# bbc/vc2-reference

Hardware: AMD Instinct MI355X
Metric: Mpixels/s encode+decode, UHD-1 10-bit HQ_ConstQ (higher is better)
Workload: dtype int32; 1 GPU; BASELINE cfg2: UHD-1 3840x2160 4:2:2 10-bit HQ_ConstQ DD97 depth 4, -u 1 -a 2 -q 16 -S 2; streams=1, parallelism=frame-parallel x1, no collective

## Files before the change

vc2-reference_amd/csrc/vc2hip_slices.hip:

```cpp
#include <stdlib.h>

#include <algorithm>
#include <atomic>
#include <mutex>

#include "vc2hip_internal.h"
#include "vc2hip_store.h"

void vc2_prof_begin(Launcher &L, const char *name, hipStream_t s);
void vc2_prof_end(Launcher &L, hipStream_t s);

__constant__ QuantTables c_qs;
void vc2_upload_p16_tables(const QuantTables &t, hipStream_t s);
void vc2_upload_tables_slices(const QuantTables &t, hipStream_t s) {
  (void)hipMemcpyToSymbolAsync(HIP_SYMBOL(c_qs), &t, sizeof t, 0, hipMemcpyHostToDevice, s);
  vc2_upload_p16_tables(t, s);
}

__device__ __forceinline__ int quant_core(int v, int qf, unsigned mg, int sh) {
  const unsigned mag = v < 0 ? 0u - (unsigned)v : (unsigned)v;
  const int a = (int)(mag << 2);
  const unsigned t = __umulhi(mg, (unsigned)a);
  int q = (int)((t + (((unsigned)a - t) >> 1)) >> sh);
  const bool slow = !(qf > 1 && a >= 0);
// ... 1946 lines not shown
      for (int c = 0; c < comp; ++c) at += 1 + (unsigned long long)rd(at) * p.scalar;
      len = rd(at) * p.scalar;
      at += 1;
      if (at + len > plen) {
        atomicOr(p.err, VC2_DEVERR_STREAM);
        len = at < plen ? (unsigned)(plen - at) : 0;
      }
      pos = at < plen ? (unsigned)at : 0u;
    }
#ifdef VC2HIP_ABLATE
    br.dbg_mask = VC2_SKIP(p, 1) ? 0x3FFCu : ~0u;
#endif
    br.safe = (unsigned)min((unsigned long long)p.payload_stride + mis, 0xFFFFFFF0ull);
    br.init(pay, pos + mis, (int)len);
  }
#pragma unroll
  for (int k = 0; k < UNP_PITCH; k += 8) *(int4 *)(st + k) = make_int4(0, 0, 0, 0);
  __syncthreads();
  int cnt = 0;
  signed char *sb = (signed char *)st;
  auto byte_of = [&](int j, int v) __attribute__((always_inline)) -> int {
    if (__builtin_expect((unsigned)(v + 127) <= 254u, 1)) return v;
    escape(j, v);
    if (p.stats) {
      const uint2 pc = *(const uint2 *)(sb + (cnt & ~7));
      auto has80 = [](unsigned x) -> bool { const unsigned y = x ^ 0x80808080u; return ((y - 0x01010101u) & ~y & 0x80808080u) != 0u; };
      if (!has80(pc.x) && !has80(pc.y)) atomicAdd(p.stats, 1ull);
    }
    return -128;
  };
  auto turns = [&](auto bytes, const int base, const int room) __attribute__((always_inline)) {
    constexpr bool BY = decltype(bytes)::value;
    for (int turn = 0; cnt < room; ++turn) {
      int used = 0;
#pragma unroll
      for (int look = 0; look < UNP_LOOKS; ++look) {
        const unsigned w = look ? (unsigned)((br.acc << used) >> 32) : br.top();
        unsigned e = lut[w >> (32 - UNP_LUT_BITS)];
#if VC2_UNP_BRANCHLESS
        if (look) e = (cnt < room && (look < 3 || used + UNP_LUT_BITS <= br.have)) ? e : 0u;
#else
        if (e != 0 && (look == 0 || (used != 0 && cnt < room)))
#endif
        {
          if constexpr (BY) {
            sb[cnt + (int)((e >> 8) & 15u)] = (signed char)(e >> 16);
            sb[cnt + (int)((e >> 12) & 15u)] = (signed char)(e >> 24);
          } else {
            st[cnt + (int)((e >> 8) & 15u)] = (short)__builtin_amdgcn_sbfe((int)e, 16, 8);
            st[cnt + (int)((e >> 12) & 15u)] = (short)((int)e >> 24);
          }
          cnt += (int)((e >> 4) & 15u);
          used += (int)(e & 15u);
        }
      }
      if ((turn & UNP_LONG_EVERY) == UNP_LONG_EVERY) {
        if (used == 0 && cnt < room) {
          const unsigned hi = br.top();
          const unsigned follow = hi & 0xAAAAAAAAu;
          if (follow != 0) {
            const int K = __clz((int)follow) >> 1;
            const unsigned body = hi >> ((32 - 2 * K) & 31);
            const unsigned mag = ((1u << K) | compact_even32(body)) - 1u;
            const int neg = (int)((hi >> ((30 - 2 * K) & 31)) & 1u);
            int v = neg ? (int)(0u - mag) : (int)mag;
            if constexpr (BY) { v = byte_of(base + cnt, v); sb[cnt++] = (signed char)v; }
            else {
              if (!St<int16_t>::fits(v)) { escape(base + cnt, v); v = VC2_ST_SENTINEL; }
              st[cnt++] = (short)v;
            }
            used = 2 * K + 2;
          } else {
            unsigned value = 1;
            for (;;) {
              const unsigned f = br.top() >> 31;
              br.skip(pay, 1);
              if (f) break;
              value = (value << 1) | (br.top() >> 31);
              br.skip(pay, 1);
            }
            value -= 1u;
            int v = 0;
            if (value) {
              v = (br.top() >> 31) ? (int)(0u - value) : (int)value;
              br.skip(pay, 1);
            }
            if constexpr (BY) { v = byte_of(base + cnt, v); sb[cnt++] = (signed char)v; }
            else {
              if (!St<int16_t>::fits(v)) { escape(base + cnt, v); v = VC2_ST_SENTINEL; }
              st[cnt++] = (short)v;
            }
          }
        }
      }
      br.skip(pay, used);
    }
  };
  const int n16 = BP8 ? min(n, p.bp.from[comp]) : n;
  int base = 0;
  for (; base < n16; base += UNP_N) {
    const int room = min(UNP_N, n - base);
    turns(std::false_type(), base, room);
    wave_lds_sync();
    const short *sw = stage[wave];
    typedef int v4i __attribute__((ext_vector_type(4)));
    typedef int v2i __attribute__((ext_vector_type(2)));
    const int rec_end = VC2_SKIP(p, 2) ? room : min(room, p.bp.from[comp] - base);
    if (rec_end > 0 && !VC2_SKIP(p, 2)) {
#pragma unroll
      for (int j = 0; j < PR; ++j) {
        const int r = j * (64 / PR) + lane / PR, c = (lane % PR) * 8;
        if (slice0 + r < p.n_slices && c < rec_end) {
          const int4 v = *(const int4 *)(sw + r * UNP_PITCH + c);
          const v4i vv = {v.x, v.y, v.z, v.w};
          int16_t *dst = (int16_t *)p.store + rec0 + (size_t)(slice0 + r) * p.slice_coefs + base + c;
          if (base + c < p.hs.n[comp])
            dst = (int16_t *)p.store + (size_t)pic * p.store_stride + (size_t)p.hs.base[comp] + (size_t)(slice0 + r) * p.hs.n[comp] + base + c;
          __builtin_nontemporal_store(vv, (__attribute__((address_space(1))) v4i *)(size_t)dst);
        }
      }
    }
    if (rec_end < room) {
      for (int q = 0; q < PR;) {
        const int j0 = base + 8 * q;
        if (8 * q >= room) break;
        if (j0 < p.bp.from[comp]) { ++q; continue; }
        int lw, ow, lbase;
        int at = band_plane_at(p.bp, comp, n, j0, sy, sx, lw, ow, &lbase);
        if (!active) at = -1;
        lw = __builtin_amdgcn_readfirstlane(lw);
        const int lp = lw - 3, P = lw >= 4 ? 1 << lp : 1;
        if (lw >= 4 && q + P <= PR && ((j0 >> 3) & (P - 1)) == 0) {
          for (int k = 0; k < P; ++k) {
            const int t = lane + 64 * k, sl = t >> lp, pp = t & (P - 1);
            const int at_t = __shfl(at, sl);
            if (at_t >= 0) {
              const int4 v = *(const int4 *)(sw + sl * UNP_PITCH + 8 * (q + pp));
              if constexpr (BP8) {
                const uint2 b8 = unp_bytes8(v, p.store_wide + (size_t)pic * p.store_stride, at_t + 8 * pp, 0, p.stats);
                const v2i vb = {(int)b8.x, (int)b8.y};
                char *dst = (char *)((int16_t *)p.store + (size_t)pic * p.store_stride) + (size_t)(at_t + 8 * pp) + (size_t)lbase;
                __builtin_nontemporal_store(vb, (__attribute__((address_space(1))) v2i *)(size_t)dst);
              } else {
              const v4i vv = {v.x, v.y, v.z, v.w};
              int16_t *dst = (int16_t *)p.store + (size_t)pic * p.store_stride + (size_t)(at_t + 8 * pp);
              __builtin_nontemporal_store(vv, (__attribute__((address_space(1))) v4i *)(size_t)dst);
              }
            }
          }
          q += P;
          continue;
        }
        if (BP8 && at >= 0) {
          const int4 v = *(const int4 *)(st + 8 * q);
          char *dst = (char *)((int16_t *)p.store + (size_t)pic * p.store_stride) + (size_t)at + (size_t)lbase;
          const uint2 b8 = unp_bytes8(v, p.store_wide + (size_t)pic * p.store_stride, at, lw >= 3 ? 0 : ow, p.stats);
          if (lw >= 3) {
            const v2i vb = {(int)b8.x, (int)b8.y};
            __builtin_nontemporal_store(vb, (__attribute__((address_space(1))) v2i *)(size_t)dst);
          } else {
            __builtin_nontemporal_store((int)b8.x, (__attribute__((address_space(1))) int *)(size_t)dst);
            __builtin_nontemporal_store((int)b8.y, (__attribute__((address_space(1))) int *)(size_t)(dst + ow));
          }
        } else if (at >= 0) {
          int16_t *dst = (int16_t *)p.store + (size_t)pic * p.store_stride + (size_t)at;
          const int4 v = *(const int4 *)(st + 8 * q);
          if (lw >= 3) {
            const v4i vv = {v.x, v.y, v.z, v.w};
            __builtin_nontemporal_store(vv, (__attribute__((address_space(1))) v4i *)(size_t)dst);
          } else {
            const v2i lo = {v.x, v.y}, hi = {v.z, v.w};
            __builtin_nontemporal_store(lo, (__attribute__((address_space(1))) v2i *)(size_t)dst);
            __builtin_nontemporal_store(hi, (__attribute__((address_space(1))) v2i *)(size_t)(dst + ow));
          }
        }
        ++q;
      }
    }
    wave_lds_sync();
    const int4 spill = *(const int4 *)(st + UNP_N);
#pragma unroll
    for (int k = 0; k < UNP_PITCH; k += 8) *(int4 *)(st + k) = make_int4(0, 0, 0, 0);
    cnt = max(cnt - UNP_N, 0);
    if (cnt) *(int4 *)st = spill;
  }
  if constexpr (BP8) {
    constexpr int UNB_N = 2 * UNP_N, UNB_PR = UNB_N / 8, UNB_PITCH = 2 * UNP_PITCH;
    static_assert(UNB_N + 8 <= UNB_PITCH, "a byte row and its slack fit the lane's part of the stage");
    if (base < n) {
      const int4 c16 = *(const int4 *)st;
      *(int4 *)st = make_int4((int)__builtin_amdgcn_perm((unsigned)c16.y, (unsigned)c16.x, 0x06040200u),
                              (int)__builtin_amdgcn_perm((unsigned)c16.w, (unsigned)c16.z, 0x06040200u), 0, 0);
    }
    const char *sw8 = (const char *)stage[wave];
    char *planes = (char *)((int16_t *)p.store + (size_t)pic * p.store_stride);
    typedef int v2i __attribute__((ext_vector_type(2)));
    for (; base < n; base += UNB_N) {
      const int room = min(UNB_N, n - base);
      turns(std::true_type(), base, room);
      wave_lds_sync();
      for (int q = 0; q < UNB_PR;) {
        if (8 * q >= room) break;
        const int j0 = base + 8 * q;
        int lw, ow, lbase;
        int at = band_plane_at(p.bp, comp, n, j0, sy, sx, lw, ow, &lbase);
        if (!active) at = -1;
        lw = __builtin_amdgcn_readfirstlane(lw);
        const int lp = lw - 3, P = lw >= 4 ? 1 << lp : 1;
        if (lw >= 4 && q + P <= UNB_PR && ((j0 >> 3) & (P - 1)) == 0) {
          for (int k = 0; k < P; ++k) {
            const int t = lane + 64 * k, sl = t >> lp, pp = t & (P - 1);
            const int at_t = __shfl(at, sl);
            if (at_t >= 0) {
              const v2i vb = *(const v2i *)(sw8 + sl * UNB_PITCH + 8 * (q + pp));
              __builtin_nontemporal_store(vb, (__attribute__((address_space(1))) v2i *)(size_t)(planes + (size_t)(at_t + 8 * pp) + (size_t)lbase));
            }
          }
          q += P;
          continue;
        }
        if (at >= 0) {
          const v2i vb = *(const v2i *)(sb + 8 * q);
          char *dst = planes + (size_t)at + (size_t)lbase;
          if (lw >= 3) __builtin_nontemporal_store(vb, (__attribute__((address_space(1))) v2i *)(size_t)dst);
          else {
            __builtin_nontemporal_store(vb.x, (__attribute__((address_space(1))) int *)(size_t)dst);
            __builtin_nontemporal_store(vb.y, (__attribute__((address_space(1))) int *)(size_t)(dst + ow));
          }
        }
        ++q;
      }
      wave_lds_sync();
      const v2i spill = *(const v2i *)(sb + UNB_N);
#pragma unroll
      for (int k = 0; k < UNB_PITCH; k += 16) *(int4 *)(sb + k) = make_int4(0, 0, 0, 0);
      cnt = max(cnt - UNB_N, 0);
      if (cnt) *(v2i *)sb = spill;
    }
  }
}

void vc2_launch_unpack(Launcher &L, const UnpackParams &p0, int n_pictures, hipStream_t s) {
  UnpackParams p = p0;
#ifdef VC2HIP_ABLATE
  { const char *e = getenv("VC2HIP_DEBUG_UNPACK"); p.debug_skip = e ? atoi(e) : 0; }
#endif
  if (!p.bp.levels) for (int c = 0; c < 3; ++c) p.bp.from[c] = 1 << 30;
  if (p.xs < 1) p.xs = 1;
  vc2_prof_begin(L, "hq_unpack", s);
  if (p.store16) {
    constexpr int T = 64 * VC2_UNP16_WAVES;
    const int nblk = (p.n_slices + T - 1) / T;
    const bool b8 = p.bp.levels && p.bp.bytes8;
#if VC2_UNP_ORDER == 2
    if (b8) VC2_LAUNCH(L, k_hq_unpack16<true>, dim3(nblk, n_pictures, 3), dim3(T), 0, s, p);
    else VC2_LAUNCH(L, k_hq_unpack16<false>, dim3(nblk, n_pictures, 3), dim3(T), 0, s, p);
#else
    if (b8) VC2_LAUNCH(L, k_hq_unpack16<true>, dim3(((nblk + 7) / 8) * 8 * 3, n_pictures), dim3(T), 0, s, p);
    else VC2_LAUNCH(L, k_hq_unpack16<false>, dim3(((nblk + 7) / 8) * 8 * 3, n_pictures), dim3(T), 0, s, p);
#endif
    vc2_prof_end(L, s);
    return;
  }
  static const int wide = vc2_tune_int("VC2HIP_UNPACK_WIDE", 1);
  static const int nt = vc2_tune_int("VC2HIP_UNPACK_NT", 1);
  if (!nt) VC2_LAUNCH(L, (k_hq_unpack<16, false>), dim3((p.n_slices + 255) / 256, n_pictures, 3), dim3(256), 0, s, p);
  else if (wide) VC2_LAUNCH(L, k_hq_unpack<32>, dim3((p.n_slices + 255) / 256, n_pictures, 3), dim3(256), 0, s, p);
  else VC2_LAUNCH(L, k_hq_unpack<16>, dim3((p.n_slices + 255) / 256, n_pictures, 3), dim3(256), 0, s, p);
  vc2_prof_end(L, s);
}

static int idx_chunk(int E) { return E <= 1024 ? 8192 : E <= 8191 ? 16384 : 32768; }

__device__ __forceinline__ int slice_len_lds(const uint8_t *b, int pos, int prefix, int scalar) {
  int q = pos + prefix + 1;
  q += 1 + b[q] * scalar;
  q += 1 + b[q] * scalar;
  q += 1 + b[q] * scalar;
  return q - pos;
}

__device__ void stage_chunk(uint8_t *lds, const uint8_t *pay, unsigned long long plen,
                            unsigned long long c0, int nbytes) {
  for (int i = threadIdx.x * 16; i < nbytes; i += blockDim.x * 16) {
    uint4 v = make_uint4(0, 0, 0, 0);
    const unsigned long long a = c0 + i;
    if (a + 16 <= plen) v = *(const uint4 *)(pay + a);
    else {
      unsigned w[4] = {0, 0, 0, 0};
      for (int k = 0; k < 16; ++k) if (a + k < plen) w[k >> 2] |= (unsigned)pay[a + k] << (8 * (k & 3));
      v = make_uint4(w[0], w[1], w[2], w[3]);
    }
    *(uint4 *)(lds + i) = v;
  }
}

static constexpr int IDX_MAX_E = 32767;
constexpr int idx_threads(int CH, int GS = 0) { return (CH >> GS) <= 8192 ? 512 : 1024; }

template <int CH, int GS>
__global__ __launch_bounds__(idx_threads(CH, GS)) void k_index_tables_nx(const uint8_t *payload, long long stride,
                                                                 const unsigned long long *lens, unsigned *tables,
                                                                 int n_chunks, int E, int prefix, int scalar, unsigned *err, const unsigned *skip,
                                                                 int merge) {
  constexpr int NT = idx_threads(CH, GS), NP = CH >> GS;
  if (skip && *skip == 0) return;
  extern __shared__ __attribute__((aligned(16))) uint8_t lds_b[];
  const int chunk = blockIdx.x, pic = blockIdx.y;
  if (chunk == 0 && threadIdx.x == 0 && lens[pic] > (unsigned long long)stride) atomicOr(err, VC2_DEVERR_STREAM);
  const unsigned long long plen = min(lens[pic], (unsigned long long)stride), c0 = (unsigned long long)chunk * CH;
  if (c0 >= plen) return;
  const int nbytes = (CH + E + 16 + 15) & ~15;
  const int EU = E >> GS;
  unsigned short *nx = (unsigned short *)(lds_b + nbytes);
  stage_chunk(lds_b, payload + (size_t)pic * stride, plen, c0, nbytes);
  __syncthreads();
  const int lim = (int)min((unsigned long long)CH, plen - c0);
  constexpr int PER = NP / NT;
  {
    int q[PER];
#pragma unroll
    for (int k = 0; k < PER; ++k) q[k] = ((threadIdx.x + k * NT) << GS) + prefix + 1;
#pragma unroll
    for (int c = 0; c < 3; ++c) {
      int len[PER];
#pragma unroll
      for (int k = 0; k < PER; ++k) len[k] = lds_b[min(q[k], nbytes - 1)];
#pragma unroll
      for (int k = 0; k < PER; ++k) q[k] += 1 + len[k] * scalar;
    }
#pragma unroll
    for (int k = 0; k < PER; ++k) {
      const int n = q[k];
      nx[threadIdx.x + k * NT] = (unsigned short)(n >= lim ? (n >= CH ? n : CH) : n);
    }
  }
  __syncthreads();
  unsigned *tab = tables + ((size_t)pic * n_chunks + chunk) * EU;
  if (!merge) {
    for (int e = threadIdx.x; e < EU; e += NT) {
      int pos = e << GS, cnt = 0;
      if (pos >= lim) pos = CH;
      while (pos < CH) { pos = nx[pos >> GS]; ++cnt; }
      tab[e] = (unsigned)(pos - CH) << 16 | (unsigned)cnt;
    }
    return;
  }
  unsigned *W = (unsigned *)(nx + NP);
  unsigned *need = W + EU;
  unsigned short *list = (unsigned short *)(need + (EU + 31) / 32);
  __shared__ unsigned s_count;
  for (int t = threadIdx.x; t < (EU + 31) / 32; t += NT) need[t] = 0;
  if (threadIdx.x == 0) s_count = 0;
  __syncthreads();
  constexpr int EPT = 4096 / NT;
  int la[EPT], ca[EPT];
#pragma unroll
  for (int k = 0; k < EPT; ++k) {
    const int e = threadIdx.x + k * NT;
    la[k] = CH; ca[k] = 0;
    if (e < EU && (e << GS) < lim) {
      int pos = e << GS, cnt = 0;
      while (pos < E) { pos = nx[pos >> GS]; ++cnt; }
      la[k] = pos; ca[k] = cnt;
      if (pos < CH) {
        const int t = (pos - E) >> GS;
        if (!(atomicOr(&need[t >> 5], 1u << (t & 31)) >> (t & 31) & 1u)) list[atomicAdd(&s_count, 1u)] = (unsigned short)t;
      }
    }
  }
  __syncthreads();
  for (int i = threadIdx.x; i < (int)s_count; i += NT) {
    const int t = list[i];
    int pos = E + (t << GS), cnt = 0;
    while (pos < CH) { pos = nx[pos >> GS]; ++cnt; }
    W[t] = (unsigned)(pos - CH) << 16 | (unsigned)cnt;
  }
  __syncthreads();
#pragma unroll
  for (int k = 0; k < EPT; ++k) {
    const int e = threadIdx.x + k * NT;
    if (e >= EU) continue;
    if (la[k] >= CH) tab[e] = (unsigned)(la[k] - CH) << 16 | (unsigned)ca[k];
    else tab[e] = W[(la[k] - E) >> GS] + (unsigned)ca[k];
  }
}

static constexpr int IDX_GROUP = 16;

template <bool WORD> __device__ __forceinline__ uint2 idx_entry(const void *tab, size_t i) {
  if constexpr (WORD) { const unsigned t = ((const unsigned *)tab)[i]; return make_uint2(t >> 16, t & 0xFFFFu); }
  else return ((const uint2 *)tab)[i];
}

template <bool WORD>
__global__ __launch_bounds__(256) void k_index_group(const unsigned long long *lens, long long stride, const void *tables,
                                                     uint2 *groups, int n_chunks, int n_groups, int E, long long span, const unsigned *skip,
                                                     int dedupe, int gsh) {
  if (skip && *skip == 0) return;
  extern __shared__ __attribute__((aligned(8))) unsigned lds_g[];
  const int g = blockIdx.x, pic = blockIdx.y;
  const unsigned long long plen = min(lens[pic], (unsigned long long)stride);
  if ((unsigned long long)g * IDX_GROUP * (unsigned long long)span >= plen) return;
  if (!dedupe) {
    for (int e = threadIdx.x; e < E; e += blockDim.x) {
      unsigned x = (unsigned)e << gsh, cnt = 0;
      for (int k = 0; k < IDX_GROUP; ++k) {
        const int c = g * IDX_GROUP + k;
        if (c >= n_chunks || (unsigned long long)c * (unsigned long long)span >= plen) break;
        const uint2 t = idx_entry<WORD>(tables, ((size_t)pic * n_chunks + c) * E + (x >> gsh));
        x = t.x;
        cnt += t.y;
      }
      groups[((size_t)pic * n_groups + g) * E + e] = make_uint2(x, cnt);
    }
    return;
  }
  unsigned *need = lds_g;
  uint2 *res = (uint2 *)(need + ((E + 1) & ~1));
  unsigned short *list = (unsigned short *)(res + E);
  __shared__ unsigned s_count;
  for (int e = threadIdx.x; e < E; e += blockDim.x) need[e] = 0;
  if (threadIdx.x == 0) s_count = 0;
  __syncthreads();
  const int c0 = g * IDX_GROUP;
  const size_t t0 = ((size_t)pic * n_chunks + c0) * E;
  for (int e = threadIdx.x; e < E; e += blockDim.x) {
    const unsigned x = idx_entry<WORD>(tables, t0 + e).x >> gsh;
    if (atomicExch(&need[x], 1u) == 0u) list[atomicAdd(&s_count, 1u)] = (unsigned short)x;
  }
  __syncthreads();
  for (int i = threadIdx.x; i < (int)s_count; i += blockDim.x) {
    unsigned x = list[i], cnt = 0;
    const unsigned x0 = x;
    for (int k = 1; k < IDX_GROUP; ++k) {
      const int c = c0 + k;
      if (c >= n_chunks || (unsigned long long)c * (unsigned long long)span >= plen) break;
      const uint2 t = idx_entry<WORD>(tables, ((size_t)pic * n_chunks + c) * E + x);
      x = t.x >> gsh;
      cnt += t.y;
    }
    res[x0] = make_uint2(x << gsh, cnt);
  }
  __syncthreads();
  for (int e = threadIdx.x; e < E; e += blockDim.x) {
    const uint2 t = idx_entry<WORD>(tables, t0 + e);
    const uint2 r = res[t.x >> gsh];
    groups[((size_t)pic * n_groups + g) * E + e] = make_uint2(r.x, t.y + r.y);
  }
}

constexpr int IDX_MAX_GROUPS = 1024;
__global__ __launch_bounds__(1024) void k_index_chain(const unsigned long long *lens, long long stride, const unsigned *tables,
                                                    const uint2 *groups, const uint2 *supers, uint2 *entries, int n_chunks,
                                                    int n_groups, int n_supers, int E, int IDX_CH, const unsigned *skip, int gsh) {
  if (skip && *skip == 0) return;
  __shared__ uint2 g_entry[IDX_MAX_GROUPS];
  __shared__ uint2 s_entry[IDX_MAX_GROUPS / IDX_GROUP];
  const int pic = blockIdx.x;
  const unsigned long long plen = min(lens[pic], (unsigned long long)stride);
  const unsigned long long gspan = (unsigned long long)IDX_GROUP * IDX_CH, sspan = gspan * IDX_GROUP;
  if (n_supers == 0) {
    if (threadIdx.x == 0) {
      unsigned entry = 0, base = 0;
      for (int g = 0; g < n_groups; ++g) {
        g_entry[g] = make_uint2(entry, base);
        if ((unsigned long long)g * gspan >= plen) continue;
        const uint2 t = groups[((size_t)pic * n_groups + g) * E + (entry >> gsh)];
        entry = t.x;
        base += t.y;
      }
    }
  } else if (threadIdx.x == 0) {
    unsigned entry = 0, base = 0;
    for (int sg = 0; sg < n_supers; ++sg) {
      s_entry[sg] = make_uint2(entry, base);
      if ((unsigned long long)sg * sspan >= plen) continue;
      const uint2 t = supers[((size_t)pic * n_supers + sg) * E + (entry >> gsh)];
      entry = t.x;
      base += t.y;
    }
  }
  __syncthreads();
  for (int sg = threadIdx.x; sg < n_supers; sg += blockDim.x) {
    unsigned entry = s_entry[sg].x, base = s_entry[sg].y;
    for (int k = 0; k < IDX_GROUP; ++k) {
      const int g = sg * IDX_GROUP + k;
      if (g >= n_groups) break;
      g_entry[g] = make_uint2(entry, base);
      if ((unsigned long long)g * gspan >= plen) continue;
      const uint2 t = groups[((size_t)pic * n_groups + g) * E + (entry >> gsh)];
      entry = t.x;
      base += t.y;
    }
  }
  __syncthreads();
  for (int g = threadIdx.x; g < n_groups; g += blockDim.x) {
    unsigned entry = g_entry[g].x, base = g_entry[g].y;
    for (int k = 0; k < IDX_GROUP; ++k) {
      const int c = g * IDX_GROUP + k;
      if (c >= n_chunks) break;
      entries[(size_t)pic * n_chunks + c] = make_uint2(entry, base);
      if ((unsigned long long)c * IDX_CH >= plen) continue;
      const unsigned t = tables[((size_t)pic * n_chunks + c) * E + (entry >> gsh)];
      entry = t >> 16;
      base += t & 0xFFFFu;
    }
  }
}

__global__ __launch_bounds__(64) void k_index_emit(const uint8_t *payload, long long stride,
                                                   const unsigned long long *lens, const uint2 *entries,
                                                   uint32_t *offsets, int n_chunks, int E, int n_slices,
                                                   int prefix, int scalar, unsigned *err, int IDX_CH, const unsigned *skip) {
  if (skip && *skip == 0) return;
  (void)E;
  const int chunk = blockIdx.x * 64 + threadIdx.x, pic = blockIdx.y;
  if (chunk >= n_chunks) return;
  const unsigned long long plen = min(lens[pic], (unsigned long long)stride), c0 = (unsigned long long)chunk * IDX_CH;
  if (c0 >= plen) return;
  const uint2 en = entries[(size_t)pic * n_chunks + chunk];
  if ((int)en.y >= n_slices || (int)en.x >= IDX_CH) return;
  const uint8_t *pay = payload + (size_t)pic * stride;
  unsigned long long pos = c0 + en.x;
  const unsigned long long end = c0 + IDX_CH;
  int k = (int)en.y;
  while (pos < end && k < n_slices) {
    offsets[(size_t)pic * n_slices + k] = (uint32_t)pos;
    if (pos >= plen) { atomicOr(err, VC2_DEVERR_STREAM); break; }
    unsigned long long q = pos + prefix + 1;
    for (int c = 0; c < 3; ++c) q += 1 + (q < plen ? (unsigned long long)pay[q] * scalar : 0ull);
    pos = q;
    ++k;
  }
}

static int idx_entries(int prefix, int scalar) { return prefix + 4 + 3 * 255 * scalar; }
static int idx_gsh(int prefix, int scalar) {
  int gsh = 0;
  while (gsh < 2 && scalar % (2 << gsh) == 0 && (prefix + 4) % (2 << gsh) == 0) ++gsh;
  return gsh;
}
#ifndef VC2_IDX_CHUNK_BY_UNITS
#define VC2_IDX_CHUNK_BY_UNITS 0
#endif
static int idx_chunk_of(int prefix, int scalar) { const int E = idx_entries(prefix, scalar); return idx_chunk(VC2_IDX_CHUNK_BY_UNITS ? std::max(E >> idx_gsh(prefix, scalar), (E + 3) / 4) : E); }

__global__ __launch_bounds__(64) void k_index_serial(const uint8_t *payload, long long stride, const unsigned long long *lens,
                                                     uint32_t *offsets, int n_slices, int prefix, int scalar, unsigned *err,
                                                     int n_pictures, const unsigned *skip) {
  if (skip && *skip == 0) return;
  const int pic = blockIdx.x * 64 + threadIdx.x;
  if (pic >= n_pictures) return;
  const uint8_t *pay = payload + (size_t)pic * stride;
  if (lens[pic] > (unsigned long long)stride) atomicOr(err, VC2_DEVERR_STREAM);
  const unsigned long long plen = min(lens[pic], (unsigned long long)stride);
  unsigned long long pos = 0;
  for (int k = 0; k < n_slices; ++k) {
    offsets[(size_t)pic * n_slices + k] = (uint32_t)pos;
    if (pos >= plen) { atomicOr(err, VC2_DEVERR_STREAM); continue; }
    unsigned long long q = pos + prefix + 1;
    for (int c = 0; c < 3; ++c) q += 1 + (q < plen ? (unsigned long long)pay[q] * scalar : 0ull);
    pos = q;
  }
}

__global__ __launch_bounds__(256) void k_cbr_index_check(const uint8_t *payload, long long stride, const unsigned long long *lens,
                                                         const int32_t *budget, const uint32_t *cbr_offs, unsigned long long total,
                                                         int n_slices, int prefix, int scalar, unsigned *bad) {
  const int slice = blockIdx.x * 256 + threadIdx.x, pic = blockIdx.y;
  if (slice >= n_slices) return;
  const uint8_t *pay = payload + (size_t)pic * stride;
  const unsigned long long plen = min(lens[pic], (unsigned long long)stride);
  bool ok = lens[pic] == total;
  unsigned long long pos = (unsigned long long)cbr_offs[slice] + prefix + 1;
  const unsigned long long end = (unsigned long long)cbr_offs[slice] + prefix + (unsigned)budget[slice];
  for (int c = 0; c < 3 && ok; ++c) {
    ok = pos < plen;
    if (ok) pos += 1 + (unsigned long long)pay[pos] * scalar;
  }
  if (!ok || pos != end || end > plen) atomicOr(bad, 1u);
}
__global__ __launch_bounds__(256) void k_cbr_index_fill(const uint32_t *cbr_offs, uint32_t *offsets, int n_slices, const unsigned *bad) {
  const int slice = blockIdx.x * 256 + threadIdx.x, pic = blockIdx.y;
  if (slice < n_slices && *bad == 0) offsets[(size_t)pic * n_slices + slice] = cbr_offs[slice];
}
void vc2_launch_cbr_index(Launcher &L, const uint8_t *payload, long long stride, const unsigned long long *lens, const int32_t *budget,
                          const uint32_t *cbr_offs, unsigned long long total, uint32_t *offsets, int n_slices, int prefix, int scalar,
                          int n_pictures, unsigned *bad, hipStream_t s) {
  vc2_prof_begin(L, "slice_index_cbr", s);
  const dim3 grid((n_slices + 255) / 256, n_pictures);
  VC2_LAUNCH(L, k_cbr_index_check, grid, dim3(256), 0, s, payload, stride, lens, budget, cbr_offs, total, n_slices, prefix, scalar, bad);
  VC2_LAUNCH(L, k_cbr_index_fill, grid, dim3(256), 0, s, cbr_offs, offsets, n_slices, bad);
  vc2_prof_end(L, s);
}

bool vc2_slice_index_supported(int prefix, int scalar);
bool vc2_slice_index_supported(int prefix, int scalar) { (void)prefix; (void)scalar; return true; }

size_t vc2_slice_index_workspace(int n_pictures, size_t max_payload, int prefix, int scalar) {
  const size_t E = idx_entries(prefix, scalar);
  if (E > (size_t)IDX_MAX_E) return 256;
  const size_t ch = (size_t)idx_chunk_of(prefix, scalar);
  const size_t n_chunks = (max_payload + ch - 1) / ch + 1;
  if (n_chunks > (size_t)1024 * 16) return 256;
  const size_t n_groups = (n_chunks + IDX_GROUP - 1) / IDX_GROUP;
  const size_t n_supers = (n_groups + IDX_GROUP - 1) / IDX_GROUP;
  return (size_t)n_pictures * (n_chunks * E * sizeof(unsigned) + (n_chunks + (n_groups + n_supers) * E) * sizeof(uint2)) + 512;
}

void vc2_launch_slice_index(Launcher &L, const uint8_t *payload, long long payload_stride,
                            const unsigned long long *lens, uint32_t *offsets, int n_slices,
                            int prefix, int scalar, int n_pictures, unsigned *err, hipStream_t s,
                            void *workspace, size_t workspace_bytes, const unsigned *skip) {
  const int E = idx_entries(prefix, scalar);
  (void)workspace_bytes;
  const bool too_many = E <= IDX_MAX_E &&
      ((size_t)payload_stride + idx_chunk_of(prefix, scalar) - 1) / idx_chunk_of(prefix, scalar) + 1 > (size_t)IDX_MAX_GROUPS * IDX_GROUP;
  if (E > IDX_MAX_E || too_many) {
    vc2_prof_begin(L, "slice_index_serial", s);
    VC2_LAUNCH(L, k_index_serial, dim3((n_pictures + 63) / 64), dim3(64), 0, s, payload, payload_stride, lens,
                       offsets, n_slices, prefix, scalar, err, n_pictures, skip);
    vc2_prof_end(L, s);
    return;
  }
  const int ch = idx_chunk_of(prefix, scalar);
  const int gsh = idx_gsh(prefix, scalar);
  const int EU = E >> gsh;
  const int n_chunks = (int)(((size_t)payload_stride + ch - 1) / ch) + 1;
  unsigned *tables = (unsigned *)workspace;
  uint2 *entries = (uint2 *)(((size_t)(tables + (size_t)n_pictures * n_chunks * EU) + 15) & ~(size_t)15);
  const size_t stage_bytes = (size_t)((ch + E + 16 + 15) & ~15);
  vc2_prof_begin(L, "slice_index_tables", s);
  {
    static const bool no_merge = vc2_tune_int("VC2HIP_IDX_NO_MERGE", 0) != 0;
    const int merge = !no_merge && EU <= 4096 && 2 * E <= ch;
    const size_t lds = stage_bytes + (size_t)(ch >> gsh) * 2 + (merge ? (size_t)EU * 6 + ((size_t)(EU + 31) / 32) * 4 + 16 : 0);
#define VC2_IDX_TABLES(CH, GS)                                                                                                    \
  do {                                                                                                                        \
    vc2_allow_lds((const void *)k_index_tables_nx<CH, GS>, lds);                                                                  \
    VC2_LAUNCH(L, (k_index_tables_nx<CH, GS>), dim3(n_chunks, n_pictures), dim3(idx_threads(CH, GS)), lds, s, payload, payload_stride, \
               lens, tables, n_chunks, E, prefix, scalar, err, skip, merge);                                                  \
  } while (0)
#define VC2_IDX_TABLES_G(CH) do { if (gsh == 0) VC2_IDX_TABLES(CH, 0); else if (gsh == 1) VC2_IDX_TABLES(CH, 1); else VC2_IDX_TABLES(CH, 2); } while (0)
    if (ch == 8192) VC2_IDX_TABLES_G(8192);
    else if (ch == 16384) VC2_IDX_TABLES_G(16384);
    else VC2_IDX_TABLES_G(32768);
#undef VC2_IDX_TABLES_G
#undef VC2_IDX_TABLES
  }
  vc2_prof_end(L, s);
  const int n_groups = (n_chunks + IDX_GROUP - 1) / IDX_GROUP;
  const int n_supers = n_groups > 128 ? (n_groups + IDX_GROUP - 1) / IDX_GROUP : 0;
  uint2 *groups = entries + (size_t)n_pictures * n_chunks;
  uint2 *supers = groups + (size_t)n_pictures * n_groups * EU;
  vc2_prof_begin(L, "slice_index_chain", s);
  {
    static const bool no_dedupe = vc2_tune_int("VC2HIP_IDX_NO_DEDUPE", 0) != 0;
    const int dedupe = !no_dedupe && EU <= 8192;
    const size_t glds = dedupe ? ((size_t)((EU + 1) & ~1) * 4 + (size_t)EU * 8 + (size_t)EU * 2 + 16) : 0;
    if (glds) { vc2_allow_lds((const void *)k_index_group<true>, glds); vc2_allow_lds((const void *)k_index_group<false>, glds); }
    VC2_LAUNCH(L, k_index_group<true>, dim3(n_groups, n_pictures), dim3(256), glds, s, lens, payload_stride, (const void *)tables, groups, n_chunks, n_groups, EU, (long long)ch, skip, dedupe, gsh);
    if (n_supers) VC2_LAUNCH(L, k_index_group<false>, dim3(n_supers, n_pictures), dim3(256), glds, s, lens, payload_stride, (const void *)groups, supers, n_groups, n_supers, EU, (long long)ch * IDX_GROUP, skip, dedupe, gsh);
  }
  VC2_LAUNCH(L, k_index_chain, dim3(n_pictures), dim3(std::min(1024, (n_groups + 63) / 64 * 64)), 0, s, lens, payload_stride, tables, groups, supers, entries, n_chunks, n_groups, n_supers, EU, ch, skip, gsh);
  vc2_prof_end(L, s);
  vc2_prof_begin(L, "slice_index_emit", s);
  VC2_LAUNCH(L, k_index_emit, dim3((n_chunks + 63) / 64, n_pictures), dim3(64), 0, s, payload,
                     payload_stride, lens, entries, offsets, n_chunks, E, n_slices, prefix, scalar, err, ch, skip);
  vc2_prof_end(L, s);
}

__device__ __forceinline__ int intlog2_dev(int value) { int l = 0; --value; while (value > 0) { value >>= 1; ++l; } return l; }

__global__ __launch_bounds__(256) void k_ld_unpack(const LdUnpackParams p) {
  constexpr int UNP_N = 32, UNP_PITCH = UNP_N + 4, LPR = UNP_N / 4;
  __shared__ __attribute__((aligned(16))) int stage[4][64 * UNP_PITCH];
  __shared__ unsigned long long outp[4][64];
  __shared__ unsigned short vlut[1024];
  const int pic = blockIdx.y;
  if (p.redo && !p.shifted[pic]) return;
  vlut_init(vlut);
  __syncthreads();
  const int lane = threadIdx.x & 63, wave = threadIdx.x >> 6;
  const int slice = blockIdx.x * 256 + threadIdx.x;
  const bool chroma = blockIdx.z != 0;
  const bool active = slice < p.n_slices;
  int *st = stage[wave] + lane * UNP_PITCH;
  const int *sw = stage[wave];
  const uint8_t *data = nullptr;
  int ystart = 0, ybits = 0, total = 0;
  long long vis = 0;
  if (active) {
    const int size = p.slice_bytes[slice];
    const unsigned off = p.redo ? p.starts[(size_t)pic * p.n_slices + slice] : p.offsets[slice];
    const long long plen = p.lens ? (long long)min(p.lens[pic], (unsigned long long)p.payload_stride) : p.payload_stride;
    vis = max(plen - (long long)off, 0ll);
    data = p.payload + (size_t)pic * p.payload_stride + min((long long)off, plen);
    unsigned head = 0;
    for (int k = 0; k < 4; ++k) head = (head << 8) | (k < min((long long)(p.redo ? 4 : size), vis) ? data[k] : 0xFFu);
    if (!chroma) p.qidx[(size_t)pic * p.n_slices + slice] = (int)(head >> 25);
    const int split = intlog2_dev(8 * size - 7);
    ybits = split ? (int)((head << 7) >> (32 - split)) : 0;
    ystart = 7 + split;
    total = 8 * size;
    if (!p.redo && p.shifted && !chroma && ybits > total - ystart) atomicOr(&p.shifted[pic], 1u);
    outp[wave][lane] = (unsigned long long)(p.store + (size_t)pic * p.store_stride + (size_t)slice * p.slice_coefs);
  } else outp[wave][lane] = 0;
  WordReader br;
  if (!chroma) {
    const int nb = p.redo ? (int)min((long long)ybits, 8 * vis - ystart) : min(ybits, total - ystart);
    if (active && nb > 0) br.init_bits(data + (ystart >> 3), ystart & 7, nb); else br.init_ones();
  }
  const int ny = chroma ? 0 : p.comp_n[0];
  for (int base = 0; base < ny; base += UNP_N) {
    const int room = min(UNP_N, ny - base);
    decode_round<UNP_N, int>(br, room, st, vlut);
    wave_lds_sync();
#pragma unroll
    for (int j = 0; j < LPR; ++j) {
      const int r = j * (64 / LPR) + lane / LPR, c = (lane % LPR) * 4;
      int32_t *rec = (int32_t *)outp[wave][r];
      if (rec && c < room) {
        const int4 v = *(const int4 *)(sw + r * UNP_PITCH + c);
        int *d = rec + p.comp_off[0] + base + c;
        typedef int v4i __attribute__((ext_vector_type(4)));
        const v4i vv = {v.x, v.y, v.z, v.w};
        __builtin_nontemporal_store(vv, (__attribute__((address_space(1))) v4i *)(size_t)d);
      }
    }
    wave_lds_sync();
  }
  if (chroma) {
    const int cstart = ystart + ybits;
    const int nb = p.redo ? (int)min((long long)(total - cstart), 8 * vis - cstart) : total - cstart;
    if (active && nb > 0 && ybits >= 0) br.init_bits(data + (cstart >> 3), cstart & 7, nb); else br.init_ones();
  }
  const int nc = chroma ? 2 * p.comp_n[1] : 0;
  for (int base = 0; base < nc; base += UNP_N) {
    const int room = min(UNP_N, nc - base);
    decode_round<UNP_N, int>(br, room, st, vlut);
    wave_lds_sync();
#pragma unroll
    for (int j = 0; j < LPR; ++j) {
      const int r = j * (64 / LPR) + lane / LPR, c = (lane % LPR) * 4;
      int32_t *rec = (int32_t *)outp[wave][r];
      if (rec && c < room) {
        const int4 v = *(const int4 *)(sw + r * UNP_PITCH + c);
        int *du = rec + p.comp_off[1] + (base + c) / 2, *dv = rec + p.comp_off[2] + (base + c) / 2;
        __builtin_nontemporal_store(v.x, du); __builtin_nontemporal_store(v.y, dv);
        if (c + 2 < room) { __builtin_nontemporal_store(v.z, du + 1); __builtin_nontemporal_store(v.w, dv + 1); }
      }
    }
    wave_lds_sync();
  }
}

void vc2_launch_ld_unpack(Launcher &L, const LdUnpackParams &p, int n_pictures, hipStream_t s) {
  vc2_prof_begin(L, "ld_unpack", s);
  VC2_LAUNCH(L, k_ld_unpack, dim3((p.n_slices + 255) / 256, n_pictures, 2), dim3(256), 0, s, p);
  vc2_prof_end(L, s);
}
__global__ __launch_bounds__(64) void k_ld_walk(const LdUnpackParams p) {
  const int pic = blockIdx.x;
  if (!p.shifted[pic] || threadIdx.x != 0) return;
  const uint8_t *pay = p.payload + (size_t)pic * p.payload_stride;
  const unsigned long long plen = p.lens ? min(p.lens[pic], (unsigned long long)p.payload_stride) : (unsigned long long)p.payload_stride;
  unsigned long long pos = 0;
  for (int si = 0; si < p.n_slices; ++si) {
    const int size = p.slice_bytes[si];
    p.starts[(size_t)pic * p.n_slices + si] = (uint32_t)min(pos, plen);
    unsigned head = 0;
    for (int k = 0; k < 4; ++k) head = (head << 8) | (pos + k < plen ? pay[pos + k] : 0xFFu);
    const int split = intlog2_dev(8 * size - 7);
    const long long ybits = split ? (long long)((head << 7) >> (32 - split)) : 0;
    const long long uvbits = 8ll * size - 7 - split - ybits;
    pos += (unsigned long long)((7 + split + ybits + max(uvbits, 0ll) + 7) >> 3);
  }
  if (pos > plen) atomicOr(p.err, VC2_DEVERR_STREAM);
}
void vc2_launch_ld_walk(Launcher &L, const LdUnpackParams &p, int n_pictures, hipStream_t s) {
  vc2_prof_begin(L, "ld_unpack", s);
  VC2_LAUNCH(L, k_ld_walk, dim3(n_pictures), dim3(64), 0, s, p);
  vc2_prof_end(L, s);
}

__global__ __launch_bounds__(1024) void k_ld_ll(const int32_t *store, long long store_stride,
                                                int slice_coefs, int coef_off, int n0, int llh, int llw,
                                                int ys, int xs, const int32_t *qidx, int qm0,
                                                int32_t *ll_plane, long long ll_stride, unsigned *err) {
  const int pic = blockIdx.x;
  const int32_t *st = store + (size_t)pic * store_stride;
  const int32_t *qi = qidx + (size_t)pic * ys * xs;
  int32_t *ll = ll_plane + (size_t)pic * ll_stride;
  const int bh = llh / ys, bw = llw / xs;
  (void)n0;
  for (int d = 0; d < llh + llw - 1; ++d) {
    const int ylo = max(0, d - (llw - 1)), yhi = min(llh - 1, d);
    for (int y = ylo + (int)threadIdx.x; y <= yhi; y += blockDim.x) {
      const int x = d - y;
      const int sv = y / bh, sh = x / bw;
      const int qv = st[(size_t)(sv * xs + sh) * slice_coefs + coef_off + (y - sv * bh) * bw + (x - sh * bw)];
      const int yb = ((y + 1) * ys - 1) / llh, xb = ((x + 1) * xs - 1) / llw;
      const int aq = max(qi[yb * xs + xb] - qm0, 0);
      if (aq > 119) atomicOr(err, VC2_DEVERR_QINDEX);
      int pred;
      if (y > 0 && x > 0) {
        const int r = ll[(size_t)(y - 1) * llw + x - 1] + ll[(size_t)(y - 1) * llw + x] + ll[(size_t)y * llw + x - 1];
        pred = r >= 0 ? (r + 1) / 3 : (r - 1) / 3;
      } else if (y > 0) pred = ll[(size_t)(y - 1) * llw + x];
      else if (x > 0) pred = ll[(size_t)y * llw + x - 1];
      else pred = 0;
      ll[(size_t)y * llw + x] = scale_dev(qv, min(aq, 119)) + pred;
    }
    __threadfence_block();
    __syncthreads();
  }
}

#ifndef VC2_LD_LL_WAVE_MAXR
#define VC2_LD_LL_WAVE_MAXR 4
#endif
template <int R> __device__ __forceinline__ void ld_ll_wave(int *rs, int llh, int llw) {
  constexpr unsigned BIAS = 0x7FFFFFFEu, BIAS3 = BIAS / 3u;
  const int lane = threadIdx.x, y0 = lane * R, nl = (llh + R - 1) / R;
  int row[R];
  bool ok[R];
  unsigned left[R], res[R];
  unsigned run = 0;
#pragma unroll
  for (int r = 0; r < R; ++r) {
    ok[r] = y0 + r < llh;
    row[r] = min(y0 + r, llh - 1) * llw;
    run += ok[r] ? (unsigned)rs[row[r]] : 0u;
    left[r] = run;
  }
  const unsigned above = (unsigned)wave_incl_scan((int)run, lane) - run;
#pragma unroll
  for (int r = 0; r < R; ++r) {
    left[r] += above;
    if (ok[r]) rs[row[r]] = (int)left[r];
    res[r] = (unsigned)rs[row[r] + min(1, llw - 1)] - BIAS3;
  }
  unsigned bottom = left[R - 1];
  unsigned prev_up = above;
  const bool top = y0 == 0;
  for (int t = 0; t < llw - 1 + nl - 1; ++t) {
    const unsigned up_in = (unsigned)dpp0<0x138, 0xf>((int)bottom);
    const int x = t - lane + 1;
    if (x >= 1 && x < llw && ok[0]) {
      unsigned nres[R];
      const int xn = min(x + 1, llw - 1);
#pragma unroll
      for (int r = 0; r < R; ++r) nres[r] = (unsigned)rs[row[r] + xn] - BIAS3;
      unsigned ul = prev_up + (BIAS + 1u), up = up_in;
#pragma unroll
      for (int r = 0; r < R; ++r) {
        unsigned d3 = __umulhi(ul + up + left[r], 0xAAAAAAABu) >> 1;
        if (r == 0) d3 = top ? left[0] + BIAS3 : d3;
        const unsigned a = res[r] + d3;
        if (ok[r]) rs[row[r] + x] = (int)a;
        ul = left[r] + (BIAS + 1u);
        left[r] = a;
        up = a;
        res[r] = nres[r];
      }
      bottom = up;
      prev_up = up_in;
    }
  }
}

__device__ __forceinline__ void ld_ll_lds_body(int pic, const int32_t *store, long long store_stride,
                                               int slice_coefs, int coef_off, int llh, int llw,
                                               int ys, int xs, const int32_t *qidx, int qm0,
                                               int32_t *ll_plane, long long ll_stride, unsigned *err) {
  extern __shared__ int rs[];
  const int32_t *st = store + (size_t)pic * store_stride;
  const int32_t *qi = qidx + (size_t)pic * ys * xs;
  const int bh = llh / ys, bw = llw / xs;
  int *qft = rs + llh * llw, *qot = qft + 120;
  for (int i = threadIdx.x; i < 120; i += blockDim.x) { qft[i] = c_qs.qf[i]; qot[i] = c_qs.off[i]; }
  __syncthreads();
  auto scale_tab = [&](int v, int qf, int qo) -> int {
    const unsigned mag = v < 0 ? 0u - (unsigned)v : (unsigned)v;
    int a = (int)(mag * (unsigned)qf);
    if (a > 0) a = (int)((unsigned)a + (unsigned)qo);
    a = (int)((unsigned)a + 2u);
    a /= 4;
    return v < 0 ? (int)(0u - (unsigned)a) : a;
  };
  const int n0 = bh * bw, ns = ys * xs;
  if (n0 <= 4) {
    for (int s0 = threadIdx.x; s0 < ns; s0 += 4 * blockDim.x) {
      int q4[4], v4[4][4];
#pragma unroll
      for (int k = 0; k < 4; ++k) {
        const int sl = min(s0 + k * (int)blockDim.x, ns - 1);
        q4[k] = qi[sl];
        const int32_t *src = st + (size_t)sl * slice_coefs + coef_off;
#pragma unroll
        for (int e = 0; e < 4; ++e) v4[k][e] = e < n0 ? src[e] : 0;
      }
#pragma unroll
      for (int k = 0; k < 4; ++k) {
        const int sl = s0 + k * (int)blockDim.x;
        if (sl >= ns) break;
        const int sv = sl / xs, sh = sl - sv * xs;
        const int aq = max(q4[k] - qm0, 0);
        if (aq > 119) atomicOr(err, VC2_DEVERR_QINDEX);
        const int qf = qft[min(aq, 119)], qo = qot[min(aq, 119)];
#pragma unroll
        for (int e = 0; e < 4; ++e)
          if (e < n0) { const int yy = e / bw, xx = e - yy * bw; rs[(sv * bh + yy) * llw + sh * bw + xx] = scale_tab(v4[k][e], qf, qo); }
      }
    }
  } else {
    for (int sl = threadIdx.x; sl < ns; sl += blockDim.x) {
      const int sv = sl / xs, sh = sl - sv * xs;
      const int aq = max(qi[sl] - qm0, 0);
      if (aq > 119) atomicOr(err, VC2_DEVERR_QINDEX);
      const int qf = qft[min(aq, 119)], qo = qot[min(aq, 119)];
      const int32_t *src = st + (size_t)sl * slice_coefs + coef_off;
      for (int yy = 0; yy < bh; ++yy)
        for (int xx = 0; xx < bw; ++xx) rs[(sv * bh + yy) * llw + sh * bw + xx] = scale_tab(src[yy * bw + xx], qf, qo);
    }
  }
  __syncthreads();
  {
    auto pred = [&](int y, int x, int ul, int up, int lf) -> int {
      if (y > 0 && x > 0) { const int r = ul + up + lf; return r >= 0 ? (r + 1) / 3 : (r - 1) / 3; }
      if (y > 0) return up;
      if (x > 0) return lf;
      return 0;
    };
    const int R = (llh + 63) / 64;
    if (R <= VC2_LD_LL_WAVE_MAXR) {
      if (threadIdx.x < 64) {
        if (R == 1) ld_ll_wave<1>(rs, llh, llw);
        else if (R == 2) ld_ll_wave<2>(rs, llh, llw);
        else if (R == 3) ld_ll_wave<3>(rs, llh, llw);
        else ld_ll_wave<4>(rs, llh, llw);
      }
      __syncthreads();
    } else
    for (int d = 0; d < (llh + 1) / 2 + (llw + 1) / 2 - 1; ++d) {
      const int nby = (llh + 1) / 2, nbx = (llw + 1) / 2;
      const int blo = max(0, d - (nbx - 1)), bhi = min(nby - 1, d);
      for (int by = blo + (int)threadIdx.x; by <= bhi; by += blockDim.x) {
        const int y0 = 2 * by, x0 = 2 * (d - by);
        const bool has_x = x0 + 1 < llw, has_y = y0 + 1 < llh;
        int *q = rs + y0 * llw + x0;
        const int w00 = y0 > 0 && x0 > 0 ? q[-llw - 1] : 0, w01 = y0 > 0 ? q[-llw] : 0, w02 = y0 > 0 && has_x ? q[-llw + 1] : 0;
        const int w10 = x0 > 0 ? q[-1] : 0, w20 = x0 > 0 && has_y ? q[llw - 1] : 0;
        const int a = (int)((unsigned)q[0] + (unsigned)pred(y0, x0, w00, w01, w10));
        q[0] = a;
        int b = 0, c = 0;
        if (has_x) { b = (int)((unsigned)q[1] + (unsigned)pred(y0, x0 + 1, w01, w02, a)); q[1] = b; }
        if (has_y) { c = (int)((unsigned)q[llw] + (unsigned)pred(y0 + 1, x0, w10, a, w20)); q[llw] = c; }
        if (has_x && has_y) q[llw + 1] = (int)((unsigned)q[llw + 1] + (unsigned)pred(y0 + 1, x0 + 1, a, b, c));
      }
      __syncthreads();
    }
  }
  int32_t *ll = ll_plane + (size_t)pic * ll_stride;
// ... 778 lines not shown
```

Baseline: 124,000 Mpixels/s.

## Follow only reachable slice-chain entries per group instead of building every chunk table

The per-chunk index table kernel now runs only on the first chunk of each group. A new k_index_follow kernel walks the remaining chunks of the group, following only the slice-start positions actually reachable from that first chunk's exits. It stages the payload in LDS sub-steps with register double-buffering of the next pieces, and writes the group transfer entries directly. This is meant to avoid computing full transition tables for every possible entry offset in most chunks. In exchange the walk inside each group becomes sequential, with more synchronisation per group.

```diff
diff --git a/vc2-reference_amd/csrc/vc2hip_slices.hip b/vc2-reference_amd/csrc/vc2hip_slices.hip
--- a/vc2-reference_amd/csrc/vc2hip_slices.hip
+++ b/vc2-reference_amd/csrc/vc2hip_slices.hip
@@ -2272,11 +2272,11 @@
 __global__ __launch_bounds__(idx_threads(CH, GS)) void k_index_tables_nx(const uint8_t *payload, long long stride,
                                                                  const unsigned long long *lens, unsigned *tables,
                                                                  int n_chunks, int E, int prefix, int scalar, unsigned *err, const unsigned *skip,
-                                                                 int merge) {
+                                                                 int merge, int chunk_step) {
   constexpr int NT = idx_threads(CH, GS), NP = CH >> GS;
   if (skip && *skip == 0) return;
   extern __shared__ __attribute__((aligned(16))) uint8_t lds_b[];
-  const int chunk = blockIdx.x, pic = blockIdx.y;
+  const int chunk = blockIdx.x * chunk_step, pic = blockIdx.y;
   if (chunk == 0 && threadIdx.x == 0 && lens[pic] > (unsigned long long)stride) atomicOr(err, VC2_DEVERR_STREAM);
   const unsigned long long plen = min(lens[pic], (unsigned long long)stride), c0 = (unsigned long long)chunk * CH;
   if (c0 >= plen) return;
@@ -2417,6 +2417,134 @@
     const uint2 t = idx_entry<WORD>(tables, t0 + e);
     const uint2 r = res[t.x >> gsh];
     groups[((size_t)pic * n_groups + g) * E + e] = make_uint2(r.x, t.y + r.y);
+  }
+}
+
+constexpr int IDX_FOLLOW_NT = 256;
+constexpr int IDX_FOLLOW_PIECES_SMALL = 3, IDX_FOLLOW_PIECES = 7;
+static size_t idx_follow_stage(int step, int E) { return (size_t)((step + E + 16 + 15) & ~15); }
+static size_t idx_follow_lds(int step, int E, int EU) { return idx_follow_stage(step, E) + (size_t)EU * 14 + ((size_t)(EU + 31) / 32) * 4; }
+
+template <int PIECES>
+__device__ __forceinline__ void idx_follow_fetch(uint4 (&piece)[PIECES], const uint8_t *pay, unsigned long long plen,
+                                                 unsigned long long base, int nbytes) {
+#pragma unroll
+  for (int p = 0; p < PIECES; ++p) {
+    const int i = (p * IDX_FOLLOW_NT + (int)threadIdx.x) * 16;
+    if (i >= nbytes) continue;
+    uint4 v = make_uint4(0, 0, 0, 0);
+    const unsigned long long a = base + i;
+    if (a + 16 <= plen) v = *(const uint4 *)(pay + a);
+    else {
+      unsigned w[4] = {0, 0, 0, 0};
+      for (int k = 0; k < 16; ++k) if (a + k < plen) w[k >> 2] |= (unsigned)pay[a + k] << (8 * (k & 3));
+      v = make_uint4(w[0], w[1], w[2], w[3]);
+    }
+    piece[p] = v;
+  }
+}
+
+template <int PIECES>
+__global__ __launch_bounds__(IDX_FOLLOW_NT) void k_index_follow(const uint8_t *payload, long long stride, const unsigned long long *lens,
+                                                                unsigned *tables, uint2 *groups, int n_chunks, int n_groups, int E,
+                                                                int prefix, int scalar, int CH, int step, const unsigned *skip, int gsh) {
+  constexpr int NT = IDX_FOLLOW_NT;
+  if (skip && *skip == 0) return;
+  extern __shared__ __attribute__((aligned(16))) uint8_t lds_f[];
+  const int g = blockIdx.x, pic = blockIdx.y, c0 = g * IDX_GROUP;
+  const unsigned long long plen = min(lens[pic], (unsigned long long)stride);
+  if ((unsigned long long)c0 * CH >= plen) return;
+  const int EU = E >> gsh, nbytes = (step + E + 16 + 15) & ~15, nsub = CH / step, nbits = (EU + 31) / 32;
+  unsigned *W = (unsigned *)(lds_f + nbytes);
+  unsigned *cnt = W + EU;
+  unsigned *need = cnt + EU;
+  unsigned short *cur = (unsigned short *)(need + nbits);
+  unsigned short *first = cur + EU;
+  unsigned short *list = first + EU;
+  __shared__ unsigned s_n[2];
+  int nfol = 0;
+  for (int k = 1; k < IDX_GROUP; ++k) {
+    const int c = c0 + k;
+    if (c >= n_chunks || (unsigned long long)c * CH >= plen) break;
+    ++nfol;
+  }
+  const uint8_t *pay = payload + (size_t)pic * stride;
+  const unsigned long long f0 = (unsigned long long)(c0 + 1) * CH;
+  const int T = nfol * nsub;
+  uint4 piece_a[PIECES], piece_b[PIECES];
+  if (T > 0) idx_follow_fetch(piece_a, pay, plen, f0, nbytes);
+  if (T > 1) idx_follow_fetch(piece_b, pay, plen, f0 + step, nbytes);
+  const unsigned *tab0 = tables + ((size_t)pic * n_chunks + c0) * EU;
+  for (int t = threadIdx.x; t < nbits; t += NT) need[t] = 0;
+  if (threadIdx.x < 2) s_n[threadIdx.x] = 0;
+  __syncthreads();
+  for (int e = threadIdx.x; e < EU; e += NT) {
+    const unsigned x = (tab0[e] >> 16) >> gsh;
+    if (!(atomicOr(&need[x >> 5], 1u << (x & 31)) >> (x & 31) & 1u)) {
+      const unsigned i = atomicAdd(&s_n[0], 1u);
+      first[i] = list[i] = (unsigned short)x;
+      cur[x] = (unsigned short)x;
+      cnt[x] = 0;
+    }
+  }
+  __syncthreads();
+  const int n1 = (int)s_n[0];
+  int n = n1;
+  auto turn = [&](uint4 (&piece)[PIECES], int t) {
+    const int k = 1 + t / nsub, j = t % nsub, c = c0 + k;
+#pragma unroll
+    for (int p = 0; p < PIECES; ++p) {
+      const int i = (p * NT + (int)threadIdx.x) * 16;
+      if (i < nbytes) *(uint4 *)(lds_f + i) = piece[p];
+    }
+    __syncthreads();
+    if (t + 2 < T) idx_follow_fetch(piece, pay, plen, f0 + (unsigned long long)(t + 2) * step, nbytes);
+    const int lim = (int)min((unsigned long long)CH, plen - (unsigned long long)c * CH);
+    const int lo = j * step, hi = lo + step;
+    const bool last = j == nsub - 1;
+    unsigned *tab = tables + ((size_t)pic * n_chunks + c) * EU;
+    for (int i = threadIdx.x; i < n; i += NT) {
+      const int x = list[i];
+      int pos, hops;
+      if (j == 0) {
+        pos = x << gsh; hops = 0;
+        if (pos >= lim) pos = CH;
+      } else {
+        const unsigned w = W[x];
+        pos = (int)(w >> 16); hops = (int)(w & 0xFFFFu);
+      }
+      while (pos < hi) {
+        const int q = pos + slice_len_lds(lds_f, pos - lo, prefix, scalar);
+        pos = q >= lim ? max(q, CH) : q;
+        ++hops;
+      }
+      const unsigned w = (unsigned)(last ? pos - CH : pos) << 16 | (unsigned)hops;
+      W[x] = w;
+      if (last) tab[x] = w;
+    }
+    if (last) for (int b = threadIdx.x; b < nbits; b += NT) need[b] = 0;
+    __syncthreads();
+    if (!last) return;
+    for (int m = threadIdx.x; m < n1; m += NT) {
+      const int x0 = first[m];
+      const unsigned w = W[cur[x0]];
+      const unsigned x = (w >> 16) >> gsh;
+      cur[x0] = (unsigned short)x;
+      cnt[x0] += w & 0xFFFFu;
+      if (!(atomicOr(&need[x >> 5], 1u << (x & 31)) >> (x & 31) & 1u)) list[atomicAdd(&s_n[k & 1], 1u)] = (unsigned short)x;
+    }
+    if (threadIdx.x == 0) s_n[(k + 1) & 1] = 0;
+    __syncthreads();
+    n = (int)s_n[k & 1];
+  };
+  for (int t = 0; t < T; t += 2) {
+    turn(piece_a, t);
+    if (t + 1 < T) turn(piece_b, t + 1);
+  }
+  for (int e = threadIdx.x; e < EU; e += NT) {
+    const unsigned t = tab0[e];
+    const unsigned x0 = (t >> 16) >> gsh;
+    groups[((size_t)pic * n_groups + g) * EU + e] = make_uint2((unsigned)cur[x0] << gsh, (t & 0xFFFFu) + cnt[x0]);
   }
 }
 
@@ -2601,6 +2729,13 @@
   unsigned *tables = (unsigned *)workspace;
   uint2 *entries = (uint2 *)(((size_t)(tables + (size_t)n_pictures * n_chunks * EU) + 15) & ~(size_t)15);
   const size_t stage_bytes = (size_t)((ch + E + 16 + 15) & ~15);
+  const int n_groups = (n_chunks + IDX_GROUP - 1) / IDX_GROUP;
+  static const bool no_dedupe = vc2_tune_int("VC2HIP_IDX_NO_DEDUPE", 0) != 0;
+  const int dedupe = !no_dedupe && EU <= 8192;
+  static const int follow_step = vc2_tune_int("VC2HIP_IDX_FOLLOW_STEP", 0);
+  const int fstep = follow_step >= 1024 && follow_step <= ch && (follow_step & (follow_step - 1)) == 0 ? follow_step : std::min(ch, 8192);
+  const bool follow = dedupe && idx_follow_stage(fstep, E) <= (size_t)IDX_FOLLOW_PIECES * IDX_FOLLOW_NT * 16 &&
+                      idx_follow_lds(fstep, E, EU) <= (size_t)64 * 1024;
   vc2_prof_begin(L, "slice_index_tables", s);
   {
     static const bool no_merge = vc2_tune_int("VC2HIP_IDX_NO_MERGE", 0) != 0;
@@ -2609,8 +2744,8 @@
 #define VC2_IDX_TABLES(CH, GS)                                                                                                    \
   do {                                                                                                                        \
     vc2_allow_lds((const void *)k_index_tables_nx<CH, GS>, lds);                                                                  \
-    VC2_LAUNCH(L, (k_index_tables_nx<CH, GS>), dim3(n_chunks, n_pictures), dim3(idx_threads(CH, GS)), lds, s, payload, payload_stride, \
-               lens, tables, n_chunks, E, prefix, scalar, err, skip, merge);                                                  \
+    VC2_LAUNCH(L, (k_index_tables_nx<CH, GS>), dim3(follow ? n_groups : n_chunks, n_pictures), dim3(idx_threads(CH, GS)), lds, s, payload, payload_stride, \
+               lens, tables, n_chunks, E, prefix, scalar, err, skip, merge, follow ? IDX_GROUP : 1);                          \
   } while (0)
 #define VC2_IDX_TABLES_G(CH) do { if (gsh == 0) VC2_IDX_TABLES(CH, 0); else if (gsh == 1) VC2_IDX_TABLES(CH, 1); else VC2_IDX_TABLES(CH, 2); } while (0)
     if (ch == 8192) VC2_IDX_TABLES_G(8192);
@@ -2620,17 +2755,26 @@
 #undef VC2_IDX_TABLES
   }
   vc2_prof_end(L, s);
-  const int n_groups = (n_chunks + IDX_GROUP - 1) / IDX_GROUP;
   const int n_supers = n_groups > 128 ? (n_groups + IDX_GROUP - 1) / IDX_GROUP : 0;
   uint2 *groups = entries + (size_t)n_pictures * n_chunks;
   uint2 *supers = groups + (size_t)n_pictures * n_groups * EU;
   vc2_prof_begin(L, "slice_index_chain", s);
   {
-    static const bool no_dedupe = vc2_tune_int("VC2HIP_IDX_NO_DEDUPE", 0) != 0;
-    const int dedupe = !no_dedupe && EU <= 8192;
     const size_t glds = dedupe ? ((size_t)((EU + 1) & ~1) * 4 + (size_t)EU * 8 + (size_t)EU * 2 + 16) : 0;
     if (glds) { vc2_allow_lds((const void *)k_index_group<true>, glds); vc2_allow_lds((const void *)k_index_group<false>, glds); }
-    VC2_LAUNCH(L, k_index_group<true>, dim3(n_groups, n_pictures), dim3(256), glds, s, lens, payload_stride, (const void *)tables, groups, n_chunks, n_groups, EU, (long long)ch, skip, dedupe, gsh);
+    if (follow) {
+      const size_t flds = idx_follow_lds(fstep, E, EU);
+#define VC2_IDX_FOLLOW(PIECES)                                                                                                  \
+  do {                                                                                                                          \
+    vc2_allow_lds((const void *)k_index_follow<PIECES>, flds);                                                                  \
+    VC2_LAUNCH(L, k_index_follow<PIECES>, dim3(n_groups, n_pictures), dim3(IDX_FOLLOW_NT), flds, s, payload, payload_stride, lens, \
+               tables, groups, n_chunks, n_groups, E, prefix, scalar, ch, fstep, skip, gsh);                                    \
+  } while (0)
+      if (idx_follow_stage(fstep, E) <= (size_t)IDX_FOLLOW_PIECES_SMALL * IDX_FOLLOW_NT * 16) VC2_IDX_FOLLOW(IDX_FOLLOW_PIECES_SMALL);
+      else VC2_IDX_FOLLOW(IDX_FOLLOW_PIECES);
+#undef VC2_IDX_FOLLOW
+    } else
+      VC2_LAUNCH(L, k_index_group<true>, dim3(n_groups, n_pictures), dim3(256), glds, s, lens, payload_stride, (const void *)tables, groups, n_chunks, n_groups, EU, (long long)ch, skip, dedupe, gsh);
     if (n_supers) VC2_LAUNCH(L, k_index_group<false>, dim3(n_supers, n_pictures), dim3(256), glds, s, lens, payload_stride, (const void *)groups, supers, n_groups, n_supers, EU, (long long)ch * IDX_GROUP, skip, dedupe, gsh);
   }
   VC2_LAUNCH(L, k_index_chain, dim3(n_pictures), dim3(std::min(1024, (n_groups + 63) / 64 * 64)), 0, s, lens, payload_stride, tables, groups, supers, entries, n_chunks, n_groups, n_supers, EU, ch, skip, gsh);
```

Measured after the change: 127,400 Mpixels/s (median of 6 runs). 2.7% higher.
